# cassiusfive/balatro-gym

Measured on AMD Instinct MI355X. Metric: env-steps/sec at 65536 envs, random policy; achieved HBM GB/s vs peak, higher is better.
Workload: dtype int64/f64

## Files before the change

### balatro_gym_amd/csrc/bg_lib.hip

```cpp
#include "../../include/balatro_mi355x.h"
#include "bg_step.h"
#include <hip/hip_ext.h>
#include <stdio.h>
#include <stdlib.h>
#include <string.h>
#include <type_traits>
#include <string>
#include <vector>


struct InfoPtrs {
  int64_t* final_score; int32_t* error; int32_t* flags; int32_t* aux; int8_t* hand_type; int8_t* cards_played;
  double* reward_terms;
  double* score_breakdown;
};

static_assert(offsetof(ObsPtrs, rows) == sizeof(bg_obs_ptrs), "the first 31 members of ObsPtrs must mirror bg_obs_ptrs");
static_assert(sizeof(InfoPtrs) == sizeof(bg_info_ptrs), "InfoPtrs must mirror bg_info_ptrs");

__device__ __forceinline__ void bg_emit_info(size_t row, const StepOut& o, uint8_t* trunc, const InfoPtrs& info) {
  if (trunc) trunc[row] = 0;
  if (info.final_score) info.final_score[row] = o.final_score;
  if (info.error) info.error[row] = o.error;
  if (info.flags) info.flags[row] = o.flags;
  if (info.aux) info.aux[row] = o.aux;
  if (info.hand_type) info.hand_type[row] = (int8_t)o.hand_type;
  if (info.cards_played) info.cards_played[row] = (int8_t)o.cards_played;
  if (info.reward_terms) {
    double2* q = (double2*)(info.reward_terms + row * 8);
#pragma unroll
    for (int i = 0; i < 4; i++) q[i] = make_double2(o.terms[2 * i], o.terms[2 * i + 1]);
  }
  if (info.score_breakdown && o.hand_type < 0) {
    double2* q = (double2*)(info.score_breakdown + row * 8);
#pragma unroll
    for (int i = 0; i < 4; i++) q[i] = make_double2(0.0, 0.0);
  }
}

#include "bg_engine.h"
#include "bg_engine3.h"

template <bool CARDS>
__global__ __launch_bounds__(BG_BLOCK) void bg_reset_kernel(BgDev d, const uint8_t* __restrict__ mask_in, ObsPtrs obs) {
  using DeckT = typename std::conditional<CARDS, Deck0C, Deck0>::type;
  int env = blockIdx.x * BG_BLOCK + threadIdx.x;
  if (env >= d.N) return;
  Env e;
  bg_load_env(d, env, e);
  DeckT dk; static_cast<Deck0&>(dk) = bg_load_deck0(d, env);
  if (!mask_in || mask_in[env]) { bg_env_reset(d, env, e, dk); bg_store_env(d, env, e); }
  ShopRegs sr; sr.valid = false;
  uint64_t mask = bg_action_mask(d, env, e, sr);
  bg_write_obs<false>(d, env, (size_t)env, e, dk, obs, mask, sr, RowExtra{0.0, 0, 0u});
}

__global__ __launch_bounds__(BG_BLOCK) void bg_observe_kernel(BgDev d, ObsPtrs obs) {
  int env = blockIdx.x * BG_BLOCK + threadIdx.x;
  if (env >= d.N) return;
  Env e;
  bg_load_env(d, env, e);
  Deck0 dk = bg_load_deck0(d, env);
  ShopRegs sr; sr.valid = false;
  uint64_t mask = bg_action_mask(d, env, e, sr);
  bg_write_obs<false>(d, env, (size_t)env, e, dk, obs, mask, sr, RowExtra{0.0, 0, 0u});
}

struct alignas(64) BgG16 { uint32_t v[16]; };
struct BgGenrandTab {
  BgG16 blk[BG_MT_N / 16];
  constexpr BgGenrandTab() : blk{} {
    uint32_t x = 19650218u;
    blk[0].v[0] = x;
    for (int i = 1; i < BG_MT_N; i++) { x = 1812433253u * (x ^ (x >> 30)) + (uint32_t)i; blk[i / 16].v[i % 16] = x; }
  }
};
static_assert(BG_MT_N % 16 == 0, "624 = 39 blocks of 16");
static constexpr BgGenrandTab BG_GENRAND{};

template <bool SLOT>
__device__ __forceinline__ void bg_mt_seed_impl(uint32_t* p, uint32_t key) {
  constexpr int NB = BG_MT_N / 16;
  uint4* p4 = (uint4*)p;
  uint32_t a = BG_GENRAND.blk[0].v[0], a1 = 0;
  {
    BgG16 cur = BG_GENRAND.blk[0];
#pragma unroll 1
    for (int b = 0; b < NB; b++) {
      const BgG16 nxt = BG_GENRAND.blk[b + 1 < NB ? b + 1 : NB - 1];
#pragma unroll
      for (int c = 0; c < 16; c++) {
        if (b > 0 || c >= 1) {
          a = (cur.v[c] ^ ((a ^ (a >> 30)) * 1664525u)) + key;
          if (b == 0 && c == 1) a1 = a;
        }
      }
      cur = nxt;
    }
  }
  const uint32_t a1w = (a1 ^ ((a ^ (a >> 30)) * 1664525u)) + key;
  a = BG_GENRAND.blk[0].v[0];
  a = (BG_GENRAND.blk[0].v[1] ^ ((a ^ (a >> 30)) * 1664525u)) + key;
  uint32_t bprev = a1w, w2 = 0, w3 = 0;
  uint32_t far0 = 0, far1 = 0, out2 = 0, out3 = 0;
  uint32_t acc = 0;
  {
    BgG16 cur = BG_GENRAND.blk[0];
#pragma unroll 1
    for (int b = 0; b < NB; b++) {
      const BgG16 nxt = BG_GENRAND.blk[b + 1 < NB ? b + 1 : NB - 1];
      uint32_t v[16];
#pragma unroll
      for (int c = 0; c < 16; c++) {
        v[c] = 0;
        if (b > 0 || c >= 2) {
          a = (cur.v[c] ^ ((a ^ (a >> 30)) * 1664525u)) + key;
          bprev = (a ^ ((bprev ^ (bprev >> 30)) * 1566083941u)) - (uint32_t)(16 * b + c);
          v[c] = bprev;
        }
      }
      if (b == 0) { w2 = v[2]; w3 = v[3]; }
      if constexpr (!SLOT) {
#pragma unroll
        for (int k = 0; k < 4; k++) {
          const int q = 4 * b + k;
          if (q == 0) continue;
          p4[q] = make_uint4(v[4 * k], v[4 * k + 1], v[4 * k + 2], v[4 * k + 3]);
        }
      } else {
        if (b < 4) {
#pragma unroll
          for (int k = 0; k < 4; k++) if (4 * b + k > 0) p4[4 * b + k] = make_uint4(v[4 * k], v[4 * k + 1], v[4 * k + 2], v[4 * k + 3]);
        } else if (b >= 24 && b <= 28) {
          const int kb = 16 * b - BG_MT_M;
          if (b == 24) { far0 = v[13]; far1 = v[14]; out2 = bg_temper(bg_twist(w2, w3, v[15])); }
          else {
            const int g0 = kb >> 2;
            uint32_t nr[20];
#pragma unroll
            for (int g = 0; g < 5; g++) {
              uint4 t = make_uint4(0u, 0u, 0u, 0u);
              if (g0 + g > 0 && g0 + g < BG_SLOT_WORDS / 4) t = p4[g0 + g];
              nr[4 * g] = t.x; nr[4 * g + 1] = t.y; nr[4 * g + 2] = t.z; nr[4 * g + 3] = t.w;
            }
            if (b == 25) nr[3] = w3;
            auto outputs = [&](auto kbc) {
              constexpr int KB = decltype(kbc)::value;
#pragma unroll
              for (int c = 0; c < 16; c++) {
                const int k = KB + c;
                if (k < BG_SW_T) {
                  const uint32_t o = bg_temper(bg_twist(nr[3 + c], nr[4 + c], v[c]));
                  if (k == 3) out3 = o; else p[k] = o;
                  if (k >= 4 && k < 24) {
                    acc |= (o >> 24) << (8 * (k & 3));
                    if ((k & 3) == 3) { p[BG_SW_PK + (k >> 2)] = acc; acc = 0u; }
                  }
                }
              }
            };
            if (b == 25) outputs(std::integral_constant<int, 16 * 25 - BG_MT_M>{});
            else if (b == 26) outputs(std::integral_constant<int, 16 * 26 - BG_MT_M>{});
            else if (b == 27) outputs(std::integral_constant<int, 16 * 27 - BG_MT_M>{});
            else outputs(std::integral_constant<int, 16 * 28 - BG_MT_M>{});
          }
        }
      }
      cur = nxt;
    }
  }
  const uint32_t w1 = (a1w ^ ((bprev ^ (bprev >> 30)) * 1566083941u)) - 1u;
  if constexpr (!SLOT) p4[0] = make_uint4(0x80000000u, w1, w2, w3);
  else {
    const uint32_t out0 = bg_temper(bg_twist(0x80000000u, w1, far0)), out1 = bg_temper(bg_twist(w1, w2, far1));
    p4[0] = make_uint4(out0, out1, out2, out3);
    static_assert(BG_SW_PK == 56 && BG_SW_SEED == 62 && BG_SLOT_WORDS == 64, "slot tail layout");
    p[BG_SW_PK] = (out0 >> 24) | ((out1 >> 24) << 8) | ((out2 >> 24) << 16) | (out3 & 0xff000000u);
    *(uint2*)(p + BG_SW_SEED) = make_uint2(key, 0u);
  }
}
__device__ void bg_mt_seed(uint32_t* __restrict__ p, uint32_t key) { bg_mt_seed_impl<false>(p, key); }
__device__ void bg_mt_seed_slot(uint32_t* __restrict__ p, uint32_t key) { bg_mt_seed_impl<true>(p, key); }

__device__ __forceinline__ uint32_t bg_q156(uint32_t q) { return q >= 156u ? q - 156u : q; }
#define BG_LAZY_U 4
#define BG_LAZY_U_SEEDRING 2
#define BG_WL_COUNTERS 32
#define BG_REFILL_WAVE_PRIO 0
template <int U = BG_LAZY_U, class F>
__device__ __forceinline__ uint32_t bg_lazy_stream(uint32_t* S, uint32_t c, bool active, F&& take) {
  uint4* S4 = (uint4*)S;
  uint32_t q = c >> 2, off = c & 3u, fq = bg_q156(q + 99u);
  uint4 a[U + 1], f[U + 1];
#pragma unroll
  for (int g = 0; g <= U; g++) { a[g] = make_uint4(0, 0, 0, 0); f[g] = a[g]; }
  if (active) {
#pragma unroll
    for (int g = 0; g <= U; g++) { a[g] = S4[bg_q156(q + (uint32_t)g)]; f[g] = S4[bg_q156(fq + (uint32_t)g)]; }
  }
#pragma unroll 1
  while (__ballot(active) != 0ull) {
    uint4 an[U], fn[U];
#pragma unroll
    for (int g = 0; g < U; g++) { an[g] = a[0]; fn[g] = a[0]; }
    if (active) {
#pragma unroll
      for (int g = 0; g < U; g++) { an[g] = S4[bg_q156(q + (uint32_t)(U + 1 + g))]; fn[g] = S4[bg_q156(fq + (uint32_t)(U + 1 + g))]; }
    }
    bool more = active;
#pragma unroll
    for (int g = 0; g < U; g++) {
      const uint4 a0 = a[g], f0 = f[g];
      const uint32_t n0 = bg_twist(a0.x, a0.y, f0.y), n1 = bg_twist(a0.y, a0.z, f0.z), n2 = bg_twist(a0.z, a0.w, f0.w), n3 = bg_twist(a0.w, a[g + 1].x, f[g + 1].x);
      const uint32_t goff = g == 0 ? off : 0u;
      uint4 o = a0;
      uint32_t used = 0;
      if (more && goff == 0u) { o.x = n0; used++; more = take(n0); }
      if (more && goff <= 1u) { o.y = n1; used++; more = take(n1); }
      if (more && goff <= 2u) { o.z = n2; used++; more = take(n2); }
      if (more) { o.w = n3; used++; more = take(n3); }
      if (used) {
        const uint32_t qg = bg_q156(q + (uint32_t)g);
        S4[qg] = o;
        if (!more) { c = 4u * qg + goff + used; if (c >= (uint32_t)BG_MT_N) c -= (uint32_t)BG_MT_N; active = false; }
      }
    }
    q = bg_q156(q + (uint32_t)U); fq = bg_q156(fq + (uint32_t)U); off = 0u;
    a[0] = a[U]; f[0] = f[U];
#pragma unroll
    for (int g = 0; g < U; g++) { a[g + 1] = an[g]; f[g + 1] = fn[g]; }
  }
  return c;
}

#define BG_MTB 16
#define BG_SSEED 128
#define BG_LAZY_SEEDED 0x80000000u
__device__ void bg_mt_twist(const uint32_t* src, uint32_t* dst) {
  uint32_t cur = src[0], first_new = 0;
  const uint4* s4 = (const uint4*)src;
  uint4* d4 = (uint4*)dst;
#pragma unroll 1
  for (int base = 0; base < BG_MT_N; base += BG_MTB) {
    uint32_t nx[BG_MTB + 4], fr[BG_MTB + 4];
#pragma unroll
    for (int g = 0; g < BG_MTB / 4 + 1; g++) { uint4 v = s4[base / 4 + g]; nx[4 * g] = v.x; nx[4 * g + 1] = v.y; nx[4 * g + 2] = v.z; nx[4 * g + 3] = v.w; }
    if (base == 224) {
#pragma unroll
      for (int j = 0; j < BG_MTB; j++) { int kk = base + j; fr[j + 1] = (kk < BG_MT_N - BG_MT_M) ? src[kk + BG_MT_M] : dst[kk + BG_MT_M - BG_MT_N]; }
    } else {
      const uint4* f4 = base < 224 ? s4 + (base + BG_MT_M - 1) / 4 : (const uint4*)dst + (base + BG_MT_M - BG_MT_N - 1) / 4;
#pragma unroll
      for (int g = 0; g < BG_MTB / 4 + 1; g++) { uint4 v = f4[g]; fr[4 * g] = v.x; fr[4 * g + 1] = v.y; fr[4 * g + 2] = v.z; fr[4 * g + 3] = v.w; }
    }
    uint32_t v[BG_MTB];
#pragma unroll
    for (int j = 0; j < BG_MTB; j++) {
      uint32_t nxt = (base + j == BG_MT_N - 1) ? first_new : nx[j + 1];
      v[j] = bg_twist(cur, nxt, fr[j + 1]);
      if (base + j == 0) first_new = v[j];
      cur = nxt;
    }
#pragma unroll
    for (int j = 0; j < BG_MTB / 4; j++) d4[base / 4 + j] = make_uint4(v[4 * j], v[4 * j + 1], v[4 * j + 2], v[4 * j + 3]);
  }
}

#include "bg_ops.h"
#include "bg_sim.h"
#include "bg_encode.h"
#include "bg_gae.h"
#include "bg_norm.h"
#include "bg_head.h"
#include "bg_ppo.h"

__global__ __launch_bounds__(BG_BLOCK) void bg_seed_kernel(BgDev d, const int64_t* __restrict__ seeds,
                                                          const uint8_t* __restrict__ mask_in, int reseed_global) {
  int env = blockIdx.x * BG_BLOCK + threadIdx.x;
  if (env >= d.N) return;
  if (mask_in && !mask_in[env]) return;
  RngWin w;
  bg_win_init(w, nullptr);
  Env e;
  bg_load_env(d, env, e);
  int64_t seed = seeds[env];
  if (reseed_global) {
    uint32_t gs = (uint32_t)((uint64_t)seed + 16000ull);
    uint32_t* g = bg_gblock(d, env, 0);
    bg_mt_seed(g, gs);
    bg_mt_twist(g, g);
    e.g_cur = 0; e.g_idx = 0; e.g_cons = 0; e.g_valid = 1;
  }
  if (seed == 0) {
    uint64_t r;
    int guard = 0;
    do {
      uint64_t lo = bg_gdraw(d, env, e, w);
      uint64_t hi = bg_gdraw(d, env, e, w) >> 31;
      r = lo | (hi << 32);
    } while (r >= 4294967296ull && ++guard < 4096);
    seed = (int64_t)(r & 0xffffffffull);
  }
  uint32_t base = (uint32_t)(uint64_t)seed;
  bg_mt_seed(bg_deckmt(d, env), base);
  bg_deckmt(d, env)[BG_MT_N] = BG_LAZY_SEEDED;
  bg_mt_seed(bg_shopgenmt(d, env), base + 2000u);
  bg_shopgenmt(d, env)[BG_MT_N] = BG_LAZY_SEEDED;
  if (d.cardmt) {
    bg_mt_seed(d.cardmt + (size_t)env * BG_MTS, base + 11000u);
    d.cardmt[(size_t)env * BG_MTS + BG_MT_N] = BG_LAZY_SEEDED;
    bg_mt_seed(d.sealmt + (size_t)env * BG_MTS, base + 13000u);
    d.sealmt[(size_t)env * BG_MTS + BG_MT_N] = BG_LAZY_SEEDED;
  }
  e.d_head = 0; e.d_cons = 0; e.d_ready = 0;
  e.s_cons = 0; e.s_ready = 0;
  d.smeta[env] = 0;
  {
    uint32_t gp = reseed_global ? 1u : (uint32_t)((e.g_cons + e.g_valid) & 0xff);
    uint32_t pv = 0u | (0u << 8) | (gp << 16) | 0x80000000u;
    d.prod_out[env] = pv;
    ((uint32_t*)d.prod_in)[env] = pv;
  }
  bg_store_env(d, env, e);
}

__global__ __launch_bounds__(BG_BLOCK) void bg_refill_zero_kernel(BgDev d) { if (threadIdx.x < BG_WL_COUNTERS) d.wl_count[threadIdx.x] = 0; }

struct BgPart { uint32_t p, q; };
__device__ __forceinline__ uint32_t bg_part_lo(uint32_t count, BgPart pt) { return (uint32_t)(((uint64_t)count * pt.p) / pt.q); }
__device__ __forceinline__ uint32_t bg_part_hi(uint32_t count, BgPart pt) { return (uint32_t)(((uint64_t)count * (pt.p + 1u)) / pt.q); }

__global__ __launch_bounds__(BG_BLOCK) void bg_refill_scan_kernel(BgDev d) {
  int env = blockIdx.x * BG_BLOCK + threadIdx.x;
  if (env >= d.N) return;
  size_t N = d.N;
  uint32_t w5 = ((const uint32_t*)&d.hot[(size_t)5 * N + env])[3];
  uint32_t w6 = ((const uint32_t*)&d.hot[(size_t)6 * N + env])[3];
  uint2 w7 = *((const uint2*)&d.hot[(size_t)7 * N + env]);
  uint32_t prod = d.prod_in[env];
  int d_cons = bg_b(w5, 3), g_cons = bg_b(w6, 3), s_cur = bg_b(w7.y, 0), s_cons = bg_b(w7.y, 1);
  int d_ready = (int)((prod - (uint32_t)d_cons) & 0xffu);
  int s_ready = (int)(((prod >> 8) - (uint32_t)s_cons) & 0xffu);
  int g_valid = (int)(((prod >> 16) - (uint32_t)g_cons) & 0xffu);
  const bool seeded = (prod >> 31) != 0;
  if (!seeded) { d.prod_out[env] = prod; return; }
  if (s_ready < d.KS - 1) {
    uint32_t sm = d.smeta[env];
    int head = (int)(sm & 0xffu), cnt = (int)((sm >> 8) & 0xffu);
    int emitted = d.KS - 1 - s_ready;
    if (emitted > cnt) emitted = cnt;
    if (emitted > 0) {
      const uint32_t base = atomicAdd(&d.wl_count[3], (uint32_t)emitted);
#pragma unroll 1
      for (int k = 0; k < emitted; k++) {
        int slot = s_cur + 1 + s_ready + k; while (slot >= d.KS) slot -= d.KS;
        d.wl_shop[2 * (size_t)(base + k)] = (uint32_t)env | ((uint32_t)slot << 24);
        d.wl_shop[2 * (size_t)(base + k) + 1] = d.sseed[(size_t)env * BG_SSEED + ((head + k) & (BG_SSEED - 1))];
      }
      head = (head + emitted) & (BG_SSEED - 1); cnt -= emitted;
    } else emitted = 0;
    if (emitted) {
      d.smeta[env] = (uint32_t)head | ((uint32_t)cnt << 8);
      prod = (prod & 0xffff00ffu) | ((((prod >> 8) + (uint32_t)emitted) & 0xffu) << 8);
    }
    if (cnt < BG_SSEED - 8) { uint32_t i = atomicAdd(&d.wl_count[1], 1u); d.wl[N + i] = (uint32_t)env; }
  }
  d.prod_out[env] = prod;
  if (d_ready < d.KD) { uint32_t i = atomicAdd(&d.wl_count[0], 1u); d.wl[i] = (uint32_t)env; }
  if (g_valid > 0 && g_valid < d.KG) { uint32_t i = atomicAdd(&d.wl_count[2], 1u); d.wl[2 * N + i] = (uint32_t)env; }
}

__global__ __launch_bounds__(BG_BLOCK) __attribute__((amdgpu_waves_per_eu(4, 4))) void bg_refill_deck_kernel(BgDev d, BgPart pt, uint32_t cursor_idx, uint32_t max_made) {
  __builtin_amdgcn_s_setprio(BG_REFILL_WAVE_PRIO);
  __shared__ uint8_t sdeck[52][BG_BLOCK];
  const size_t N = d.N;
  const int tid = threadIdx.x;
  const uint32_t count0 = d.wl_count[0], lo = bg_part_lo(count0, pt), count = bg_part_hi(count0, pt);
  uint32_t* const cursor = &d.wl_count[cursor_idx];
  const int cap = max_made ? (int)max_made : 1 << 30;
  int env = 0, d_head = 0, d_ready = 0, made = 0;
  uint32_t prod = 0, cur = 0;
  uint32_t* mt = bg_deckmt(d, 0);
  bool have = false, need = false, dry = false;
#pragma unroll 1
  while (true) {
    if (!dry) {
      const unsigned long long freem = __ballot(!have);
      if (freem != 0ull) {
        const int leader = __ffsll(freem) - 1, nfree = __popcll(freem);
        uint32_t base = 0;
        if (tid == leader) base = atomicAdd(cursor, (uint32_t)nfree);
        base = lo + (uint32_t)__shfl((int)base, leader);
        dry = base + (uint32_t)nfree >= count;
        const uint32_t my = base + (uint32_t)__popcll(freem & ((1ull << tid) - 1ull));
        if (!have && my < count) {
          env = (int)d.wl[my];
          mt = bg_deckmt(d, env);
          const uint32_t w5 = ((const uint32_t*)&d.hot[(size_t)5 * N + env])[3];
          prod = d.prod_out[env];
          d_head = bg_b(w5, 2);
          d_ready = (int)((prod - (uint32_t)bg_b(w5, 3)) & 0xffu);
          cur = mt[BG_MT_N] & 0x3ffu;
          made = 0;
          need = d_ready < d.KD;
          have = need;
        }
      }
    }
    if (__ballot(need) == 0ull) { if (dry) break; continue; }
    if (need) { int p = 0; for (int s = 0; s < 4; s++) for (int r = 0; r < 13; r++) sdeck[p++][tid] = (uint8_t)(r * 4 + s); }
    int i = 51;
    cur = bg_lazy_stream(mt, cur, need, [&](uint32_t y) {
      const int k = 32 - __clz((uint32_t)(i + 1));
      const uint32_t j = bg_temper(y) >> (32 - k);
      if (j <= (uint32_t)i) {
        const uint8_t a = sdeck[i][tid], b = sdeck[j][tid];
        sdeck[i][tid] = b; sdeck[j][tid] = a;
        i--;
      }
      return i >= 1;
    });
    if (need) {
      const int slot = (d_head + d_ready) % d.KD;
#pragma unroll
      for (int k = 0; k < BG_NDECK; k++) {
        uint32_t wv[4] = {0, 0, 0, 0};
#pragma unroll
        for (int b = 0; b < 16; b++) { int i2 = k * 16 + b; if (i2 < 52) wv[b >> 2] |= (uint32_t)sdeck[i2][tid] << (8 * (b & 3)); }
        d.ndeck[((size_t)slot * BG_NDECK + k) * N + env] = make_uint4(wv[0], wv[1], wv[2], wv[3]);
      }
      d_ready++; made++;
      need = d_ready < d.KD && made < cap;
      if (!need) {
        mt[BG_MT_N] = cur | BG_LAZY_SEEDED;
        ((uint8_t*)&d.prod_out[env])[0] = (uint8_t)((prod + (uint32_t)made) & 0xffu);
        have = false;
      }
    }
  }
}

__global__ __launch_bounds__(BG_BLOCK) void bg_refill_seedring_kernel(BgDev d, BgPart pt) {
  __builtin_amdgcn_s_setprio(BG_REFILL_WAVE_PRIO);
  size_t N = d.N;
  const uint32_t count0 = d.wl_count[1], lo = bg_part_lo(count0, pt), count = bg_part_hi(count0, pt);
  for (uint32_t base = lo + blockIdx.x * BG_BLOCK; base < count; base += gridDim.x * BG_BLOCK) {
    const bool valid = base + threadIdx.x < count;
    const int env = valid ? (int)d.wl[N + base + threadIdx.x] : 0;
    uint32_t* mt = bg_shopgenmt(d, env);
    int head = 0, cnt = BG_SSEED;
    uint32_t cur = 0;
    if (valid) {
      const uint32_t sm = d.smeta[env];
      head = (int)(sm & 0xffu); cnt = (int)((sm >> 8) & 0xffu);
      cur = mt[BG_MT_N] & 0x3ffu;
    }
    const bool need = valid && cnt < BG_SSEED;
    cur = bg_lazy_stream<BG_LAZY_U_SEEDRING>(mt, cur, need, [&](uint32_t y) {
      const uint32_t r = bg_temper(y);
      if (r < 2147483648u) { d.sseed[(size_t)env * BG_SSEED + ((head + cnt) & (BG_SSEED - 1))] = r; cnt++; }
      return cnt < BG_SSEED;
    });
    if (need) {
      mt[BG_MT_N] = cur | BG_LAZY_SEEDED;
      d.smeta[env] = (uint32_t)head | ((uint32_t)cnt << 8);
    }
  }
}

__global__ __launch_bounds__(BG_BLOCK, 8) void bg_refill_shop_kernel(BgDev d, BgPart pt) {
  const uint32_t count0 = d.wl_count[3], lo = bg_part_lo(count0, pt), count = bg_part_hi(count0, pt);
  for (uint32_t item = lo + blockIdx.x * BG_BLOCK + threadIdx.x; item < count; item += gridDim.x * BG_BLOCK) {
    uint32_t es = d.wl_shop[2 * (size_t)item], seed = d.wl_shop[2 * (size_t)item + 1];
    bg_mt_seed_slot(bg_sblock(d, (int)(es & 0xffffffu), (int)(es >> 24)), seed);
  }
}
__global__ __launch_bounds__(BG_BLOCK) void bg_refill_gblk_kernel(BgDev d, BgPart pt) {
  __builtin_amdgcn_s_setprio(BG_REFILL_WAVE_PRIO);
  const size_t N = d.N;
  const uint32_t count0 = d.wl_count[2], lo = bg_part_lo(count0, pt), count = bg_part_hi(count0, pt);
  const int l = threadIdx.x;
  constexpr int NR = (BG_MT_N + 63) / 64;
  for (uint32_t item = lo + blockIdx.x; item < count; item += gridDim.x) {
    const int env = (int)d.wl[2 * N + item];
    const uint32_t w6 = ((const uint32_t*)&d.hot[(size_t)6 * N + env])[3];
    const uint32_t prod = d.prod_out[env];
    const int g_cur = bg_b(w6, 2), g_cons = bg_b(w6, 3);
    int g_valid = (int)(((prod >> 16) - (uint32_t)g_cons) & 0xffu);
    if (g_valid <= 0 || g_valid >= d.KG) continue;
    int last = (g_cur + g_valid - 1) % d.KG, made = 0;
    uint32_t o[NR + 1];
    {
      const uint32_t* src = bg_gblock(d, env, last);
#pragma unroll
      for (int r = 0; r < NR; r++) o[r] = (64 * r + l < BG_MT_N) ? __builtin_nontemporal_load(&src[64 * r + l]) : 0u;
      o[NR] = 0u;
    }
#pragma unroll 1
    while (g_valid < d.KG) {
      const int nxt = last + 1 == d.KG ? 0 : last + 1;
      uint32_t* dst = bg_gblock(d, env, nxt);
      uint32_t n[NR];
#pragma unroll
      for (int r = 0; r < NR; r++) {
        const int k = 64 * r + l;
        const uint32_t up_same = __shfl(o[r], (l + 1) & 63), up_next = __shfl(o[r + 1], 0);
        uint32_t up = l == 63 ? up_next : up_same;
        if (r == NR - 1) { const uint32_t new0 = __shfl(n[0], 0); if (k == BG_MT_N - 1) up = new0; }
        uint32_t far = 0u;
        if (64 * r < BG_MT_N - BG_MT_M) {
          const uint32_t a = r + 6 < NR ? __shfl(o[r + 6], (l + 13) & 63) : 0u, b2 = r + 7 < NR ? __shfl(o[r + 7], (l + 13) & 63) : 0u;
          far = l + 13 < 64 ? a : b2;
        }
        if (64 * r + 63 >= BG_MT_N - BG_MT_M) {
          const uint32_t a = r >= 4 ? __shfl(n[r >= 4 ? r - 4 : 0], (l + 29) & 63) : 0u, b2 = r >= 3 ? __shfl(n[r >= 3 ? r - 3 : 0], (l + 29) & 63) : 0u;
          const uint32_t fn = l + 29 < 64 ? a : b2;
          if (k >= BG_MT_N - BG_MT_M) far = fn;
        }
        n[r] = bg_twist(o[r], up, far);
        if (k < BG_MT_N) __builtin_nontemporal_store(n[r], &dst[k]);
      }
      if (l < 16) bg_gblock(d, env, last)[BG_MT_N + l] = n[0];
#pragma unroll
      for (int r = 0; r < NR; r++) o[r] = n[r];
      last = nxt; g_valid++; made++;
    }
    if (made && l == 0) {
      const uint32_t g = ((prod >> 16) + (uint32_t)made) & 0xffu;
      ((uint8_t*)&d.prod_out[env])[2] = (uint8_t)g;
    }
  }
}

__global__ __launch_bounds__(BG_BLOCK) void bg_inject_kernel(BgDev d, const uint8_t* __restrict__ mask_in) {
  int env = blockIdx.x * BG_BLOCK + threadIdx.x;
  if (env >= d.N) return;
  if (mask_in && !mask_in[env]) return;
  Env e;
  bg_load_env(d, env, e);
  uint4 t0 = d.tmpl[env], t1 = d.tmpl[(size_t)d.N + env];
  if (t0.y & 0x80000000u) { e.njokers = (int)bg_b(t0.y, 1); e.jokers = (uint64_t)t0.x | ((uint64_t)(t0.y & 0xffu) << 32); }
  if (t0.y & 0x40000000u) e.money = (int32_t)t0.z;
  if (t0.y & 0x20000000u) e.ante = (int)bg_b(t0.y, 2);
  if (t0.y & 0x10000000u) { e.levels = (uint64_t)t1.x | ((uint64_t)(t1.y & 0xffffu) << 32); e.excess = 0; }
  if (t1.z & 0x80000000u) { e.ncons = (int)bg_b(t1.z, 0); e.cons0 = bg_b(t1.z, 1); e.cons1 = bg_b(t1.z, 2); }
  bg_store_env(d, env, e);
}

__global__ __launch_bounds__(256) void bg_tables_build_kernel(uint32_t* out) {
  __shared__ JTables jt;
  { uint32_t* w = (uint32_t*)&jt; for (int i = threadIdx.x; i < (int)(sizeof(JTables) / 4); i += blockDim.x) w[i] = 0u; }
  __syncthreads();
  bg_tables_init(&jt);
  const uint32_t* w = (const uint32_t*)&jt;
  for (int i = threadIdx.x; i < (int)(sizeof(JTables) / 4); i += blockDim.x) out[i] = w[i];
}

__global__ __launch_bounds__(BG_BLOCK) void bg_inject_deck_kernel(BgDev d, const uint4* __restrict__ decks, const uint8_t* __restrict__ mask_in) {
  int env = blockIdx.x * BG_BLOCK + threadIdx.x;
  if (env >= d.N) return;
  if (mask_in && !mask_in[env]) return;
#pragma unroll
  for (int k = 0; k < BG_NDECK; k++) d.deck[(size_t)k * d.N + env] = decks[(size_t)env * BG_NDECK + k];
}
__global__ __launch_bounds__(BG_BLOCK) void bg_set_cap_kernel(BgDev d, const int32_t* __restrict__ caps, int scalar, const uint8_t* __restrict__ mask_in) {
  int env = blockIdx.x * BG_BLOCK + threadIdx.x;
  if (env >= d.N) return;
  if (mask_in && !mask_in[env]) return;
  uint32_t* w = ((uint32_t*)&d.hot[(size_t)7 * d.N + env]) + 3;
  const int cap = caps ? caps[env] : scalar;
  *w = (*w & 0xffffu) | ((uint32_t)(cap & 0xff) << 16);
}

struct bg_handle {
  BgDev dev;
  int device_id;
  bool seeded;
  int64_t* d_seeds;
  uint8_t* d_mask;
  uint32_t* d_jtab;
  int steps_since_refill;
  std::vector<uint4> h_tmpl;
  std::vector<hipEvent_t> ev_pool;
  std::vector<uint8_t> h_cap;
  uint64_t bytes;
  std::string err;
  bool profiling;
  uint32_t* d_prod[2];
  long refill_seq;
  long refill_done;
  long view_min;
  bool async_refill;
  hipStream_t side;
  hipEvent_t ev_refill[2];
  hipEvent_t ev_rollout;
  std::vector<hipEvent_t> ev_rollout_t, ev_refill_t, ev_step_t;
  std::vector<int> rollout_steps;
  struct RefillPiece { int kind; uint32_t part, nparts; int grid; uint32_t cursor, max_made; };
  std::vector<RefillPiece> pieces;
  size_t piece_next;
  BgDev piece_dev;
  int refill_sliced, piece_parts[4], deck_passes;
  uint32_t eng_smask; int eng_copiers;
  int engine;
  int e3_cfg, e3_epw;
  uint8_t* gpeer[8]; uint8_t** d_gpeer; int gworld, grank;
};

static std::string g_create_err;

struct BgDeviceGuard {
  int prev = -1;
  bool switched = false;
  explicit BgDeviceGuard(int dev) {
    if (hipGetDevice(&prev) == hipSuccess && prev != dev) switched = hipSetDevice(dev) == hipSuccess;
  }
  ~BgDeviceGuard() { if (switched) (void)hipSetDevice(prev); }
};
#define BG_GUARD(h) BgDeviceGuard _guard((h)->device_id)

#define BG_HIP(call)                                                                                   \
  do {                                                                                                 \
    hipError_t _e = (call);                                                                            \
    if (_e != hipSuccess) {                                                                            \
      h->err = std::string(#call) + ": " + hipGetErrorString(_e);                                      \
      return BG_E_HIP;                                                                                 \
    }                                                                                                  \
// ... 872 lines not shown
  v.push_back({d.sseed, 1, BG_SSEED * 4}); v.push_back({d.smeta, 1, 4});
  v.push_back({bg_prod_latest(h), 1, 4});
  if (d.cstate) { v.push_back({d.cstate, BG_NCST, 16}); v.push_back({d.ctmpl, BG_NCST, 16}); v.push_back({d.cardmt, 1, (size_t)BG_MTS * 4}); v.push_back({d.sealmt, 1, (size_t)BG_MTS * 4}); }
}
uint64_t bg_state_blob_bytes(const bg_handle* h) {
  if (!h) return 0;
  std::vector<BgSlice> v;
  bg_slices(const_cast<bg_handle*>(h), v);
  uint64_t b = 16;
  for (auto& s : v) b += s.rows * s.elem;
  return b;
}
#define BG_BLOB_MAGIC 0x42474d58u
#define BG_BLOB_VERSION 7u
static int bg_blob_args(bg_handle* h, const char* fn, int env_index, const void* blob, uint64_t blob_bytes) {
  if (!h) return BG_E_ARG;
  char buf[200];
  if (!blob) { h->err = std::string(fn) + ": null blob"; return BG_E_ARG; }
  if (env_index < 0 || env_index >= h->dev.N) { snprintf(buf, sizeof(buf), "%s: env_index %d out of range [0, %d)", fn, env_index, h->dev.N); h->err = buf; return BG_E_ARG; }
  const uint64_t want = bg_state_blob_bytes(h);
  if (blob_bytes < want) {
    snprintf(buf, sizeof(buf), "%s: blob of %llu bytes, this handle's blobs are %llu bytes (ring depths and card-state flag decide the size)", fn,
             (unsigned long long)blob_bytes, (unsigned long long)want);
    h->err = buf; return BG_E_ARG;
  }
  return 0;
}
int bg_get_state(bg_handle* h, int env_index, void* blob_host, uint64_t blob_bytes) {
  int rc = bg_blob_args(h, "bg_get_state", env_index, blob_host, blob_bytes);
  if (rc) return rc;
  BG_GUARD(h);
  rc = bg_refill_pieces(h, 1 << 30);
  if (rc) return rc;
  BG_HIP(hipDeviceSynchronize());
  uint8_t* out = (uint8_t*)blob_host;
  uint32_t hdr[4] = {BG_BLOB_MAGIC, BG_BLOB_VERSION, (uint32_t)h->dev.KG | (h->dev.cstate ? 0x10000u : 0u), (uint32_t)h->dev.KS | ((uint32_t)h->dev.KD << 16)};
  memcpy(out, hdr, 16); out += 16;
  std::vector<BgSlice> v;
  bg_slices(h, v);
  size_t N = h->dev.N;
  for (auto& s : v) {
    BG_HIP(hipMemcpy2D(out, s.elem, (uint8_t*)s.base + (size_t)env_index * s.elem, N * s.elem, s.elem, s.rows, hipMemcpyDeviceToHost));
    out += s.rows * s.elem;
  }
  return 0;
}
int bg_set_state(bg_handle* h, int env_index, const void* blob_host, uint64_t blob_bytes) {
  int rc = bg_blob_args(h, "bg_set_state", env_index, blob_host, blob_bytes);
  if (rc) return rc;
  BG_GUARD(h);
  const uint8_t* in = (const uint8_t*)blob_host;
  uint32_t hdr[4];
  memcpy(hdr, in, 16); in += 16;
  char buf[200];
  if (hdr[0] != BG_BLOB_MAGIC) { h->err = "bg_set_state: not a state blob (bad magic)"; return BG_E_ARG; }
  if (hdr[1] != BG_BLOB_VERSION) { snprintf(buf, sizeof(buf), "bg_set_state: blob version %u, this library reads version %u", hdr[1], BG_BLOB_VERSION); h->err = buf; return BG_E_ARG; }
  if (hdr[2] != ((uint32_t)h->dev.KG | (h->dev.cstate ? 0x10000u : 0u)) || hdr[3] != ((uint32_t)h->dev.KS | ((uint32_t)h->dev.KD << 16))) {
    snprintf(buf, sizeof(buf), "bg_set_state: the blob was saved with ring depths %u/%u/%u%s, this handle has %d/%d/%d%s", hdr[2] & 0xffffu, hdr[3] & 0xffffu, hdr[3] >> 16,
             (hdr[2] & 0x10000u) ? " + card states" : "", h->dev.KG, h->dev.KS, h->dev.KD, h->dev.cstate ? " + card states" : "");
    h->err = buf; return BG_E_ARG;
  }
  rc = bg_refill_pieces(h, 1 << 30);
  if (rc) return rc;
  BG_HIP(hipDeviceSynchronize());
  std::vector<BgSlice> v;
  bg_slices(h, v);
  size_t N = h->dev.N;
  for (auto& s : v) {
    BG_HIP(hipMemcpy2D((uint8_t*)s.base + (size_t)env_index * s.elem, N * s.elem, in, s.elem, s.elem, s.rows, hipMemcpyHostToDevice));
    if (s.base == (void*)h->dev.tmpl)
      for (size_t r = 0; r < s.rows; r++) memcpy(&h->h_tmpl[r * N + (size_t)env_index], in + r * s.elem, sizeof(uint4));
    if (s.base == (void*)h->dev.hot) { uint4 c7; memcpy(&c7, in + 7 * s.elem, sizeof(uint4)); h->h_cap[env_index] = (uint8_t)((c7.w >> 16) & 0xffu); }
    in += s.rows * s.elem;
  }
  {
    uint32_t w = 0;
    BG_HIP(hipMemcpy(&w, bg_prod_latest(h) + env_index, 4, hipMemcpyDeviceToHost));
    BG_HIP(hipMemcpy(h->d_prod[0] + env_index, &w, 4, hipMemcpyHostToDevice));
    BG_HIP(hipMemcpy(h->d_prod[1] + env_index, &w, 4, hipMemcpyHostToDevice));
  }
  h->seeded = true;
  h->steps_since_refill = 1 << 30;
  return 0;
}

int bg_inject_deck(bg_handle* h, const uint8_t* decks_host, const uint8_t* mask_host, void* stream) {
  if (!h || !decks_host) return BG_E_ARG;
  BG_GUARD(h);
  hipStream_t s = (hipStream_t)stream;
  const size_t N = h->dev.N;
  std::vector<uint8_t> packed(N * 64, 0);
  for (size_t i = 0; i < N; i++) {
    if (mask_host && !mask_host[i]) continue;
    uint64_t seen = 0;
    for (int c = 0; c < 52; c++) {
      const uint8_t v = decks_host[i * 52 + c];
      if (v >= 52 || ((seen >> v) & 1ull)) { h->err = "bg_inject_deck: every deck must be a permutation of the 52 card codes (rank-2)*4+suit"; return BG_E_ARG; }
      seen |= 1ull << v;
      packed[i * 64 + c] = v;
    }
  }
  uint4* dd = nullptr;
  BG_HIP(hipMalloc((void**)&dd, packed.size()));
  BG_HIP(hipMemcpyAsync(dd, packed.data(), packed.size(), hipMemcpyHostToDevice, s));
  if (mask_host) BG_HIP(hipMemcpyAsync(h->d_mask, mask_host, N, hipMemcpyHostToDevice, s));
  { int rcw = bg_wait_refill(h, s, 0); if (rcw) { (void)hipFree(dd); return rcw; } }
  hipLaunchKernelGGL(bg_inject_deck_kernel, dim3(bg_grid(h)), dim3(BG_BLOCK), 0, s, h->dev, (const uint4*)dd,
                     mask_host ? (const uint8_t*)h->d_mask : (const uint8_t*)nullptr);
  BG_HIP(hipGetLastError());
  BG_HIP(hipStreamSynchronize(s));
  BG_HIP(hipFree(dd));
  return 0;
}

int bg_set_max_ante(bg_handle* h, int max_ante, const int32_t* per_env_host, const uint8_t* mask_host, void* stream) {
  if (!h) return BG_E_ARG;
  BG_GUARD(h);
  hipStream_t s = (hipStream_t)stream;
  const size_t N = h->dev.N;
  if (!per_env_host && (max_ante < 0 || max_ante > 255)) { h->err = "bg_set_max_ante: the cap must be in [0, 255] (0 = none)"; return BG_E_ARG; }
  int32_t* dc = nullptr;
  for (size_t i = 0; i < N; i++) {
    if (mask_host && !mask_host[i]) continue;
    const int c = per_env_host ? per_env_host[i] : max_ante;
    if (c < 0 || c > 255) { h->err = "bg_set_max_ante: every cap must be in [0, 255] (0 = none)"; return BG_E_ARG; }
    const uint32_t ty = h->h_tmpl[i].y;
    if (c > 0 && ((ty >> 24) & 0x20u) && (int)((ty >> 16) & 0xffu) > c) { h->err = "bg_set_max_ante: a cap below the env's template ante (bg_inject)"; return BG_E_ARG; }
  }
  for (size_t i = 0; i < N; i++)
    if (!mask_host || mask_host[i]) h->h_cap[i] = (uint8_t)(per_env_host ? per_env_host[i] : max_ante);
  if (per_env_host) {
    BG_HIP(hipMalloc((void**)&dc, N * sizeof(int32_t)));
    BG_HIP(hipMemcpyAsync(dc, per_env_host, N * sizeof(int32_t), hipMemcpyHostToDevice, s));
  }
  if (mask_host) BG_HIP(hipMemcpyAsync(h->d_mask, mask_host, N, hipMemcpyHostToDevice, s));
  hipLaunchKernelGGL(bg_set_cap_kernel, dim3(bg_grid(h)), dim3(BG_BLOCK), 0, s, h->dev, (const int32_t*)dc, max_ante,
                     mask_host ? (const uint8_t*)h->d_mask : (const uint8_t*)nullptr);
  BG_HIP(hipGetLastError());
  BG_HIP(hipStreamSynchronize(s));
  if (dc) BG_HIP(hipFree(dc));
  if (!per_env_host && !mask_host) h->dev.max_ante = max_ante;
  return 0;
}

#define BG_HIP0(call)                                                                                  \
  do {                                                                                                 \
    hipError_t _e = (call);                                                                            \
    if (_e != hipSuccess) {                                                                            \
      g_create_err = std::string(#call) + ": " + hipGetErrorString(_e);                                \
      return BG_E_HIP;                                                                                 \
    }                                                                                                  \
  } while (0)

typedef uint32_t bg_cp_u32x4 __attribute__((ext_vector_type(4)));
__global__ __launch_bounds__(256) void bg_stream_copy_kernel(const bg_cp_u32x4* __restrict__ src, bg_cp_u32x4* __restrict__ dst, size_t n16) {
  const size_t i = (size_t)blockIdx.x * 256 * 4 + threadIdx.x;
  bg_cp_u32x4 v[4];
#pragma unroll
  for (int k = 0; k < 4; k++) if (i + (size_t)k * 256 < n16) v[k] = __builtin_nontemporal_load(&src[i + (size_t)k * 256]);
#pragma unroll
  for (int k = 0; k < 4; k++) if (i + (size_t)k * 256 < n16) __builtin_nontemporal_store(v[k], &dst[i + (size_t)k * 256]);
}
int bg_bench_copy(const void* src_dev, void* dst_dev, uint64_t bytes, int iters, double* gbps_out, void* stream) {
  if (!src_dev || !dst_dev || !gbps_out || bytes < 16 || iters < 1 || ((uintptr_t)src_dev & 15) || ((uintptr_t)dst_dev & 15)) { g_create_err = "bg_bench_copy: bad arguments"; return BG_E_ARG; }
  hipStream_t s = (hipStream_t)stream;
  const size_t n16 = bytes / 16;
  const unsigned grid = (unsigned)((n16 + 1023) / 1024);
  hipEvent_t a, b;
  BG_HIP0(hipEventCreate(&a)); BG_HIP0(hipEventCreate(&b));
  for (int i = 0; i < 2; i++) hipLaunchKernelGGL(bg_stream_copy_kernel, dim3(grid), dim3(256), 0, s, (const bg_cp_u32x4*)src_dev, (bg_cp_u32x4*)dst_dev, n16);
  BG_HIP0(hipEventRecord(a, s));
  for (int i = 0; i < iters; i++) hipLaunchKernelGGL(bg_stream_copy_kernel, dim3(grid), dim3(256), 0, s, (const bg_cp_u32x4*)src_dev, (bg_cp_u32x4*)dst_dev, n16);
  BG_HIP0(hipEventRecord(b, s));
  BG_HIP0(hipGetLastError());
  BG_HIP0(hipEventSynchronize(b));
  float ms = 0;
  BG_HIP0(hipEventElapsedTime(&ms, a, b));
  (void)hipEventDestroy(a); (void)hipEventDestroy(b);
  *gbps_out = ms > 0 ? 2.0 * (double)(n16 * 16) * iters / (ms * 1e-3) / 1e9 : 0.0;
  return 0;
}

__global__ __launch_bounds__(256) void bg_stream_fill_kernel(uint4* __restrict__ dst, size_t n16, uint32_t seed) {
  const size_t i = (size_t)blockIdx.x * 256 + threadIdx.x;
  if (i < n16) dst[i] = make_uint4(seed, (uint32_t)i, 0u, seed ^ (uint32_t)i);
}
int bg_bench_fill(void* dst_dev, uint64_t bytes, int iters, double* gbps_out, void* stream) {
  if (!dst_dev || !gbps_out || bytes < 16 || iters < 1 || ((uintptr_t)dst_dev & 15)) { g_create_err = "bg_bench_fill: bad arguments"; return BG_E_ARG; }
  hipStream_t s = (hipStream_t)stream;
  const size_t n16 = bytes / 16;
  const unsigned grid = (unsigned)((n16 + 255) / 256);
  hipEvent_t a, b;
  BG_HIP0(hipEventCreate(&a)); BG_HIP0(hipEventCreate(&b));
  for (int i = 0; i < 2; i++) hipLaunchKernelGGL(bg_stream_fill_kernel, dim3(grid), dim3(256), 0, s, (uint4*)dst_dev, n16, 0u);
  BG_HIP0(hipEventRecord(a, s));
  for (int i = 0; i < iters; i++) hipLaunchKernelGGL(bg_stream_fill_kernel, dim3(grid), dim3(256), 0, s, (uint4*)dst_dev, n16, (uint32_t)i + 1u);
  BG_HIP0(hipEventRecord(b, s));
  BG_HIP0(hipGetLastError());
  BG_HIP0(hipEventSynchronize(b));
  float ms = 0;
  BG_HIP0(hipEventElapsedTime(&ms, a, b));
  (void)hipEventDestroy(a); (void)hipEventDestroy(b);
  *gbps_out = ms > 0 ? (double)(n16 * 16) * iters / (ms * 1e-3) / 1e9 : 0.0;
  return 0;
}

struct BgOpTimer {
  hipEvent_t a = nullptr, b = nullptr;
  bool on = false;
  int begin(float* out, hipStream_t s) { on = out != nullptr; if (!on) return 0; BG_HIP0(hipEventCreate(&a)); BG_HIP0(hipEventCreate(&b)); BG_HIP0(hipEventRecord(a, s)); return 0; }
  void mark(hipStream_t s) { if (on) (void)hipEventRecord(b, s); }
  int end(float* out) { if (!on) return 0; BG_HIP0(hipEventSynchronize(b)); BG_HIP0(hipEventElapsedTime(out, a, b)); (void)hipEventDestroy(a); (void)hipEventDestroy(b); return 0; }
};

int bg_classify_batch_ex(const uint8_t* cards_dev, const uint8_t* n_dev, uint8_t* hand_type_dev, int64_t m, int lanes_per_case,
                         float* kernel_ms_out, void* stream) {
  if (!cards_dev || !n_dev || !hand_type_dev || m < 0 || ((uintptr_t)cards_dev & 7) || (lanes_per_case != 1 && lanes_per_case != 8)) {
    g_create_err = "bg_classify_batch: bad arguments (cards_dev must be 8-byte aligned, lanes_per_case 1 or 8)"; return BG_E_ARG;
  }
  if (kernel_ms_out) *kernel_ms_out = 0.f;
  if (m == 0) return 0;
  hipStream_t s = (hipStream_t)stream;
  BgOpTimer tm;
  int rc = tm.begin(kernel_ms_out, s);
  if (rc) return rc;
  if (lanes_per_case == 1)
    hipLaunchKernelGGL(bg_classify_batch_kernel, dim3((unsigned)((m + BG_BLOCK - 1) / BG_BLOCK)), dim3(BG_BLOCK), 0, s, cards_dev, n_dev, hand_type_dev, (long long)m);
  else
    hipLaunchKernelGGL(bg_classify_batch_l8_kernel, dim3((unsigned)((m * 8 + BG_BLOCK - 1) / BG_BLOCK)), dim3(BG_BLOCK), 0, s, cards_dev, n_dev, hand_type_dev, (long long)m);
  tm.mark(s);
  BG_HIP0(hipGetLastError());
  return tm.end(kernel_ms_out);
}
int bg_classify_batch(const uint8_t* cards_dev, const uint8_t* n_dev, uint8_t* hand_type_dev, int64_t m, void* stream) {
  return bg_classify_batch_ex(cards_dev, n_dev, hand_type_dev, m, 1, nullptr, stream);
}

int bg_encode_cols(int layout) { const int d = bg_enc_cols(layout); return d > 0 ? d : BG_E_ARG; }

int bg_encode_rows(const uint8_t* rows_dev, uint64_t row_stride_bytes, int64_t m, int layout, int out_dtype, void* out_dev,
                   uint64_t out_stride_elems, float* kernel_ms_out, void* stream) {
  const int D = bg_enc_cols(layout);
  const uint64_t es = out_dtype == BG_ENC_F32 ? 4u : 2u;
  const char* bad = nullptr;
  if (D < 0) bad = "layout must be BG_ENC_PRODUCED, BG_ENC_FIXED or BG_ENC_EXTRACTOR";
  else if (out_dtype != BG_ENC_F32 && out_dtype != BG_ENC_BF16) bad = "out_dtype must be BG_ENC_F32 or BG_ENC_BF16";
  else if (m < 0 || m > (int64_t)BG_ENC_RECS * 0x7fffffffll) bad = "m out of range";
  else if (const char* r = bg_rows_args(rows_dev, row_stride_bytes)) bad = r;
  else if (!out_dev || ((uintptr_t)out_dev & (es - 1))) bad = "out_dev must be a device pointer aligned to its element type";
  else if (out_stride_elems < (uint64_t)D || out_stride_elems > 0xffffffffull) bad = "out_stride_elems must be >= the layout's column count";
  if (bad) { g_create_err = std::string("bg_encode_rows: ") + bad; return BG_E_ARG; }
  if (kernel_ms_out) *kernel_ms_out = 0.f;
  if (m == 0) return 0;
  const bool base16 = ((uintptr_t)out_dev & 15) == 0;
  const int st = base16 && (out_stride_elems * es) % 16 == 0 ? BG_ENC_ST_ROWS : base16 && out_stride_elems == (uint64_t)D ? BG_ENC_ST_FLAT : BG_ENC_ST_ELEM;
  const unsigned grid = (unsigned)((m + BG_ENC_RECS - 1) / BG_ENC_RECS);
  hipStream_t s = (hipStream_t)stream;
  BgOpTimer tm;
  int rc = tm.begin(kernel_ms_out, s);
  if (rc) return rc;
#define BG_ENC_GO(L, T) bg_encode_launch<L, T>(st, grid, s, rows_dev, row_stride_bytes, (long long)m, out_dev, out_stride_elems)
  if (out_dtype == BG_ENC_F32) { if (layout == BG_ENC_PRODUCED) BG_ENC_GO(BG_ENC_PRODUCED, BG_ENC_F32); else if (layout == BG_ENC_FIXED) BG_ENC_GO(BG_ENC_FIXED, BG_ENC_F32); else BG_ENC_GO(BG_ENC_EXTRACTOR, BG_ENC_F32); }
  else { if (layout == BG_ENC_PRODUCED) BG_ENC_GO(BG_ENC_PRODUCED, BG_ENC_BF16); else if (layout == BG_ENC_FIXED) BG_ENC_GO(BG_ENC_FIXED, BG_ENC_BF16); else BG_ENC_GO(BG_ENC_EXTRACTOR, BG_ENC_BF16); }
#undef BG_ENC_GO
  tm.mark(s);
  BG_HIP0(hipGetLastError());
  return tm.end(kernel_ms_out);
}

static const char* bg_scan_args(const uint8_t* rows_dev, uint64_t row_stride_bytes, int K, int64_t N) {
  if (K < 0 || N < 0 || N > (int64_t)BG_GAE_ENVS * 0x7fffffffll) return "K / N out of range";
  return bg_rows_args(rows_dev, row_stride_bytes);
}

int bg_gae_rows_ex(const uint8_t* rows_dev, uint64_t row_stride_bytes, int K, int64_t N, const float* values_dev, const float* last_values_dev,
                   double gamma, double gae_lambda, float* advantages_dev, float* returns_dev, const double* rewards_dev, float* kernel_ms_out, void* stream) {
  const char* const who = rewards_dev ? "bg_gae_rows_ex: " : "bg_gae_rows: ";
  const char* bad = bg_scan_args(rows_dev, row_stride_bytes, K, N);
  if (!bad && (!values_dev || !last_values_dev || !advantages_dev)) bad = "values_dev, last_values_dev and advantages_dev must be device pointers";
  else if (!bad && (((uintptr_t)values_dev | (uintptr_t)last_values_dev | (uintptr_t)advantages_dev | (uintptr_t)returns_dev) & 3)) bad = "float arrays must be 4-byte aligned";
  else if (!bad && ((uintptr_t)rewards_dev & 7)) bad = "rewards_dev must be 8-byte aligned";
  else if (!bad && (advantages_dev == values_dev || returns_dev == values_dev || (returns_dev && returns_dev == advantages_dev))) bad = "advantages_dev / returns_dev must not be the same pointer as values_dev or as each other";
  else if (!bad && rewards_dev && ((const void*)rewards_dev == (const void*)advantages_dev || (const void*)rewards_dev == (const void*)returns_dev)) bad = "advantages_dev / returns_dev must not be the same pointer as rewards_dev";
  if (bad) { g_create_err = std::string(who) + bad; return BG_E_ARG; }
  if (kernel_ms_out) *kernel_ms_out = 0.f;
  if (K == 0 || N == 0) return 0;
  const unsigned grid = (unsigned)((N + BG_GAE_ENVS - 1) / BG_GAE_ENVS);
  const float g = bg_gae_g(gamma), gl = bg_gae_gl(gamma, gae_lambda);
  hipStream_t s = (hipStream_t)stream;
  BgOpTimer tm;
  int rc = tm.begin(kernel_ms_out, s);
  if (rc) return rc;
#define BG_GAE_GO(R, W) hipLaunchKernelGGL((bg_gae_kernel<R, W>), dim3(grid), dim3(BG_GAE_BLOCK), 0, s, rows_dev, row_stride_bytes, K, (long long)N, values_dev, last_values_dev, g, gl, advantages_dev, returns_dev, rewards_dev)
  if (returns_dev) { if (rewards_dev) BG_GAE_GO(true, true); else BG_GAE_GO(true, false); }
  else { if (rewards_dev) BG_GAE_GO(false, true); else BG_GAE_GO(false, false); }
#undef BG_GAE_GO
  tm.mark(s);
  BG_HIP0(hipGetLastError());
  return tm.end(kernel_ms_out);
}
int bg_gae_rows(const uint8_t* rows_dev, uint64_t row_stride_bytes, int K, int64_t N, const float* values_dev, const float* last_values_dev,
                double gamma, double gae_lambda, float* advantages_dev, float* returns_dev, float* kernel_ms_out, void* stream) {
  return bg_gae_rows_ex(rows_dev, row_stride_bytes, K, N, values_dev, last_values_dev, gamma, gae_lambda, advantages_dev, returns_dev, nullptr, kernel_ms_out, stream);
}

int bg_episode_stats_rows(const uint8_t* rows_dev, uint64_t row_stride_bytes, int K, int64_t N, double* ep_return_carry_dev, int32_t* ep_len_carry_dev,
                          double* ep_return_dev, int32_t* ep_len_dev, float* kernel_ms_out, void* stream) {
// ... 392 lines not shown
```

Measured before the change: 7.781 billion.

## Compute MT slot outputs in registers instead of reloading state from memory

Result: faster. 8.031 billion, median of 6 (+3.2%).

```diff
diff --git a/balatro_gym_amd/csrc/bg_lib.hip b/balatro_gym_amd/csrc/bg_lib.hip
--- a/balatro_gym_amd/csrc/bg_lib.hip
+++ b/balatro_gym_amd/csrc/bg_lib.hip
@@ -78,6 +78,13 @@
 static_assert(BG_MT_N % 16 == 0, "624 = 39 blocks of 16");
 static constexpr BgGenrandTab BG_GENRAND{};
 
+#if defined(__HIP_DEVICE_COMPILE__)
+typedef uint32_t bg_u32x4v __attribute__((ext_vector_type(4)));
+__device__ __forceinline__ void bg_store16(uint4* dst, uint32_t x, uint32_t y, uint32_t z, uint32_t w) { bg_u32x4v v; v.x = x; v.y = y; v.z = z; v.w = w; *(bg_u32x4v*)dst = v; }
+#else
+__device__ __forceinline__ void bg_store16(uint4* dst, uint32_t x, uint32_t y, uint32_t z, uint32_t w) { *dst = make_uint4(x, y, z, w); }
+#endif
+
 template <bool SLOT>
 __device__ __forceinline__ void bg_mt_seed_impl(uint32_t* p, uint32_t key) {
   constexpr int NB = BG_MT_N / 16;
@@ -102,67 +109,80 @@
   a = BG_GENRAND.blk[0].v[0];
   a = (BG_GENRAND.blk[0].v[1] ^ ((a ^ (a >> 30)) * 1664525u)) + key;
   uint32_t bprev = a1w, w2 = 0, w3 = 0;
-  uint32_t far0 = 0, far1 = 0, out2 = 0, out3 = 0;
-  uint32_t acc = 0;
+  uint32_t da = 0, db = 0, far0 = 0, far1 = 0, out2 = 0, out3 = 0, acc = 0;
+  uint32_t og[4] = {0, 0, 0, 0}, pk[5] = {0, 0, 0, 0, 0};
+  static_assert(BG_SW_T == 56 && BG_SW_PK == 56 && BG_SW_SEED == 62 && BG_SLOT_WORDS == 64, "slot layout: 14 groups of outputs, packed words 0..3, packed words 4 5 + seed + padding");
   {
     BgG16 cur = BG_GENRAND.blk[0];
+    auto slot_block = [&](auto bc) {
+      constexpr int B = decltype(bc)::value;
+#pragma unroll
+      for (int c = 0; c < 16; c++) {
+        a = (cur.v[c] ^ ((a ^ (a >> 30)) * 1664525u)) + key;
+        bprev = (a ^ ((bprev ^ (bprev >> 30)) * 1566083941u)) - (uint32_t)(16 * B + c);
+        const int k = 16 * B + c - BG_MT_M;
+        if (k == 0) far0 = bprev;
+        if (k == 1) {
+          far1 = bprev;
+          da = BG_GENRAND.blk[0].v[0];
+          da = (BG_GENRAND.blk[0].v[1] ^ ((da ^ (da >> 30)) * 1664525u)) + key;
+          db = a1w;
+        }
+        if (k >= 1 && k < BG_SW_T) {
+          const int i = k + 1;
+          const uint32_t sk = db;
+          da = (BG_GENRAND.blk[i / 16].v[i % 16] ^ ((da ^ (da >> 30)) * 1664525u)) + key;
+          db = (da ^ ((db ^ (db >> 30)) * 1566083941u)) - (uint32_t)i;
+          if (k == 1) w2 = db;
+          else {
+            const uint32_t o = bg_temper(bg_twist(sk, db, bprev));
+            if (k == 2) out2 = o;
+            else if (k == 3) out3 = o;
+            else {
+              og[k & 3] = o;
+              if ((k & 3) == 3) bg_store16(p4 + (k >> 2), og[0], og[1], og[2], og[3]);
+              if (k < 24) {
+                acc |= (o >> 24) << (8 * (k & 3));
+                if ((k & 3) == 3) {
+                  if ((k >> 2) == 5) bg_store16(p4 + BG_SLOT_WORDS / 4 - 1, pk[4], acc, key, 0u);
+                  else pk[k >> 2] = acc;
+                  acc = 0u;
+                }
+              }
+            }
+          }
+        }
+      }
+    };
 #pragma unroll 1
     for (int b = 0; b < NB; b++) {
       const BgG16 nxt = BG_GENRAND.blk[b + 1 < NB ? b + 1 : NB - 1];
-      uint32_t v[16];
-#pragma unroll
-      for (int c = 0; c < 16; c++) {
-        v[c] = 0;
-        if (b > 0 || c >= 2) {
-          a = (cur.v[c] ^ ((a ^ (a >> 30)) * 1664525u)) + key;
-          bprev = (a ^ ((bprev ^ (bprev >> 30)) * 1566083941u)) - (uint32_t)(16 * b + c);
-          v[c] = bprev;
+      bool slot_blk = false;
+      if constexpr (SLOT) slot_blk = b >= 24 && b <= 28;
+      if (slot_blk) {
+        if (b == 24) slot_block(std::integral_constant<int, 24>{});
+        else if (b == 25) slot_block(std::integral_constant<int, 25>{});
+        else if (b == 26) slot_block(std::integral_constant<int, 26>{});
+        else if (b == 27) slot_block(std::integral_constant<int, 27>{});
+        else slot_block(std::integral_constant<int, 28>{});
+      } else {
+        uint32_t v[16];
+#pragma unroll
+        for (int c = 0; c < 16; c++) {
+          v[c] = 0;
+          if (b > 0 || c >= 2) {
+            a = (cur.v[c] ^ ((a ^ (a >> 30)) * 1664525u)) + key;
+            bprev = (a ^ ((bprev ^ (bprev >> 30)) * 1566083941u)) - (uint32_t)(16 * b + c);
+            v[c] = bprev;
+          }
         }
-      }
-      if (b == 0) { w2 = v[2]; w3 = v[3]; }
-      if constexpr (!SLOT) {
-#pragma unroll
-        for (int k = 0; k < 4; k++) {
-          const int q = 4 * b + k;
-          if (q == 0) continue;
-          p4[q] = make_uint4(v[4 * k], v[4 * k + 1], v[4 * k + 2], v[4 * k + 3]);
-        }
-      } else {
-        if (b < 4) {
-#pragma unroll
-          for (int k = 0; k < 4; k++) if (4 * b + k > 0) p4[4 * b + k] = make_uint4(v[4 * k], v[4 * k + 1], v[4 * k + 2], v[4 * k + 3]);
-        } else if (b >= 24 && b <= 28) {
-          const int kb = 16 * b - BG_MT_M;
-          if (b == 24) { far0 = v[13]; far1 = v[14]; out2 = bg_temper(bg_twist(w2, w3, v[15])); }
-          else {
-            const int g0 = kb >> 2;
-            uint32_t nr[20];
-#pragma unroll
-            for (int g = 0; g < 5; g++) {
-              uint4 t = make_uint4(0u, 0u, 0u, 0u);
-              if (g0 + g > 0 && g0 + g < BG_SLOT_WORDS / 4) t = p4[g0 + g];
-              nr[4 * g] = t.x; nr[4 * g + 1] = t.y; nr[4 * g + 2] = t.z; nr[4 * g + 3] = t.w;
-            }
-            if (b == 25) nr[3] = w3;
-            auto outputs = [&](auto kbc) {
-              constexpr int KB = decltype(kbc)::value;
-#pragma unroll
-              for (int c = 0; c < 16; c++) {
-                const int k = KB + c;
-                if (k < BG_SW_T) {
-                  const uint32_t o = bg_temper(bg_twist(nr[3 + c], nr[4 + c], v[c]));
-                  if (k == 3) out3 = o; else p[k] = o;
-                  if (k >= 4 && k < 24) {
-                    acc |= (o >> 24) << (8 * (k & 3));
-                    if ((k & 3) == 3) { p[BG_SW_PK + (k >> 2)] = acc; acc = 0u; }
-                  }
-                }
-              }
-            };
-            if (b == 25) outputs(std::integral_constant<int, 16 * 25 - BG_MT_M>{});
-            else if (b == 26) outputs(std::integral_constant<int, 16 * 26 - BG_MT_M>{});
-            else if (b == 27) outputs(std::integral_constant<int, 16 * 27 - BG_MT_M>{});
-            else outputs(std::integral_constant<int, 16 * 28 - BG_MT_M>{});
+        if constexpr (!SLOT) {
+          if (b == 0) { w2 = v[2]; w3 = v[3]; }
+#pragma unroll
+          for (int k = 0; k < 4; k++) {
+            const int q = 4 * b + k;
+            if (q == 0) continue;
+            p4[q] = make_uint4(v[4 * k], v[4 * k + 1], v[4 * k + 2], v[4 * k + 3]);
           }
         }
       }
@@ -173,10 +193,8 @@
   if constexpr (!SLOT) p4[0] = make_uint4(0x80000000u, w1, w2, w3);
   else {
     const uint32_t out0 = bg_temper(bg_twist(0x80000000u, w1, far0)), out1 = bg_temper(bg_twist(w1, w2, far1));
-    p4[0] = make_uint4(out0, out1, out2, out3);
-    static_assert(BG_SW_PK == 56 && BG_SW_SEED == 62 && BG_SLOT_WORDS == 64, "slot tail layout");
-    p[BG_SW_PK] = (out0 >> 24) | ((out1 >> 24) << 8) | ((out2 >> 24) << 16) | (out3 & 0xff000000u);
-    *(uint2*)(p + BG_SW_SEED) = make_uint2(key, 0u);
+    bg_store16(p4, out0, out1, out2, out3);
+    bg_store16(p4 + BG_SW_PK / 4, (out0 >> 24) | ((out1 >> 24) << 8) | ((out2 >> 24) << 16) | (out3 & 0xff000000u), pk[1], pk[2], pk[3]);
   }
 }
 __device__ void bg_mt_seed(uint32_t* __restrict__ p, uint32_t key) { bg_mt_seed_impl<false>(p, key); }
@@ -370,6 +388,7 @@
   if (g_valid > 0 && g_valid < d.KG) { uint32_t i = atomicAdd(&d.wl_count[2], 1u); d.wl[2 * N + i] = (uint32_t)env; }
 }
 
+typedef uint32_t bg_cp_u32x4 __attribute__((ext_vector_type(4)));
 __global__ __launch_bounds__(BG_BLOCK) __attribute__((amdgpu_waves_per_eu(4, 4))) void bg_refill_deck_kernel(BgDev d, BgPart pt, uint32_t cursor_idx, uint32_t max_made) {
   __builtin_amdgcn_s_setprio(BG_REFILL_WAVE_PRIO);
   __shared__ uint8_t sdeck[52][BG_BLOCK];
@@ -427,7 +446,8 @@
         uint32_t wv[4] = {0, 0, 0, 0};
 #pragma unroll
         for (int b = 0; b < 16; b++) { int i2 = k * 16 + b; if (i2 < 52) wv[b >> 2] |= (uint32_t)sdeck[i2][tid] << (8 * (b & 3)); }
-        d.ndeck[((size_t)slot * BG_NDECK + k) * N + env] = make_uint4(wv[0], wv[1], wv[2], wv[3]);
+        bg_cp_u32x4 nv; nv.x = wv[0]; nv.y = wv[1]; nv.z = wv[2]; nv.w = wv[3];
+        __builtin_nontemporal_store(nv, (bg_cp_u32x4*)&d.ndeck[((size_t)slot * BG_NDECK + k) * N + env]);
       }
       d_ready++; made++;
       need = d_ready < d.KD && made < cap;
@@ -471,8 +491,8 @@
 __global__ __launch_bounds__(BG_BLOCK, 8) void bg_refill_shop_kernel(BgDev d, BgPart pt) {
   const uint32_t count0 = d.wl_count[3], lo = bg_part_lo(count0, pt), count = bg_part_hi(count0, pt);
   for (uint32_t item = lo + blockIdx.x * BG_BLOCK + threadIdx.x; item < count; item += gridDim.x * BG_BLOCK) {
-    uint32_t es = d.wl_shop[2 * (size_t)item], seed = d.wl_shop[2 * (size_t)item + 1];
-    bg_mt_seed_slot(bg_sblock(d, (int)(es & 0xffffffu), (int)(es >> 24)), seed);
+    const uint2 it = ((const uint2*)d.wl_shop)[item];
+    bg_mt_seed_slot(bg_sblock(d, (int)(it.x & 0xffffffu), (int)(it.x >> 24)), it.y);
   }
 }
 __global__ __launch_bounds__(BG_BLOCK) void bg_refill_gblk_kernel(BgDev d, BgPart pt) {
@@ -1651,7 +1671,6 @@
     }                                                                                                  \
   } while (0)
 
-typedef uint32_t bg_cp_u32x4 __attribute__((ext_vector_type(4)));
 __global__ __launch_bounds__(256) void bg_stream_copy_kernel(const bg_cp_u32x4* __restrict__ src, bg_cp_u32x4* __restrict__ dst, size_t n16) {
   const size_t i = (size_t)blockIdx.x * 256 * 4 + threadIdx.x;
   bg_cp_u32x4 v[4];
```
